# danpovey/quantization

Measured on AMD Instinct MI355X. Metric: vectors encoded/sec at dim=512, 8 codebooks; uint8 codes bit-exact vs ref, higher is better.
Workload: dtype f32 (products: exact 30-bit fixed point on the i8 MFMA); 1 GPU; Quantizer.encode, dim=512, bytes_per_frame=8, codebook_size=256, refine_indexes_iters=5, batch=65536 fp32 Gaussian vectors per GPU (BASELINE.json configs[1]), seeded synthetic codebooks; global_batch=65536, parallelism=batch-sharded x1, no collective

## Files before the change

include/mcq.h:

```cpp
#ifndef MCQ_H
#define MCQ_H

#include <stddef.h>
#include <stdint.h>

#ifdef __cplusplus
extern "C" {
#endif

#define MCQ_EINVAL (-1)
#define MCQ_EUNSUPPORTED (-2)
#define MCQ_EWORKSPACE (-3)

#define MCQ_ABI_VERSION 7
int mcq_abi_version(void);

int mcq_padded_dim(int D);

size_t mcq_prepared_bytes(int N, int K, int D);
size_t mcq_prepared_decode_bytes(int N, int K, int D);
size_t mcq_prepared_mean_offset(int N, int K, int D);
int mcq_prepare(const float *centers, float cscale_exp, const float *weight, const float *bias,
                int N, int K, int D, void *prepared, void *stream);

int mcq_prepare_dev(const float *centers, const float *scales_exp, const float *weight, const float *bias,
                    int N, int K, int D, void *prepared, void *stream);

int mcq_prepare_params(const float *centers, const float *centers_scale, const float *logits_scale, float speed,
                       const float *weight, const float *bias, int N, int K, int D, void *prepared,
                       float *scales_exp_out, void *stream);

size_t mcq_encode_workspace_bytes(long B, int N, int K, int D);
int mcq_encode(const float *x, long B, const void *prepared, float lscale_exp, int N, int K, int D,
               int refine_iters, uint8_t *out_u8, int64_t *out_i64, void *workspace,
               size_t workspace_bytes, void *stream);

#define MCQ_ENCODE_SKIP_FIXED_POINTS 1u
#define MCQ_ENCODE_ALL_PASSES 8u
#define MCQ_ENCODE_LSCALE_FROM_PREPARED 2u
#define MCQ_ENCODE_X_FP16 4u
int mcq_encode_ex(const float *x, long B, const void *prepared, float lscale_exp, int N, int K, int D,
                  int refine_iters, uint8_t *out_u8, int64_t *out_i64, void *workspace,
                  size_t workspace_bytes, void *stream, unsigned flags);

int mcq_refine_indexes(const float *x, long B, const void *prepared, int N, int K, int D, int refine_iters,
                       const int64_t *idx_in, int64_t *idx_out, void *workspace, size_t workspace_bytes,
                       void *stream);

int mcq_decode(const void *codes, int code_bytes, int codes_per_row, long B, const void *prepared,
               int N, int K, int D, float *out, void *stream);

int mcq_decode_backward(const float *grad_out, const int64_t *idx, long B, int N, int K, int D, float *gC,
                        void *stream);

int mcq_logits_argmax(const float *x, long B, const void *prepared, float lscale_exp, int N, int K, int D,
                      float *logits_out, int64_t *argmax_out, void *workspace, size_t workspace_bytes,
                      void *stream, unsigned flags);

int mcq_logits_refine(const float *x, long B, const void *prepared, float lscale_exp, int N, int K, int D,
                      int refine_iters, float *logits_out, int64_t *idx_out, void *workspace, size_t workspace_bytes,
                      void *stream, unsigned flags);
int mcq_logits_refine_codes(const float *x, long B, const void *prepared, float lscale_exp, int N, int K, int D,
                            int refine_iters, float *logits_out, int64_t *idx_out, uint8_t *codes_out, void *workspace,
// ... 81 lines not shown
```

quantization_amd/_lib.py:

```python
import ctypes
import os

_HERE = os.path.dirname(os.path.abspath(__file__))
_ALT = os.environ.get("MCQ_LIB_PATH") if os.environ.get("MCQ_ALLOW_LIB_PATH") == "1" else None
LIB_PATH = _ALT or os.path.join(_HERE, "lib", "libmcq_hip.so")

SYMBOLS = (
    "mcq_abi_version", "mcq_padded_dim", "mcq_prepared_bytes", "mcq_prepared_decode_bytes", "mcq_prepared_mean_offset", "mcq_prepare", "mcq_prepare_dev", "mcq_prepare_params", "mcq_encode_workspace_bytes",
    "mcq_encode", "mcq_encode_ex", "mcq_refine_indexes", "mcq_decode", "mcq_decode_backward", "mcq_logits", "mcq_logits_workspace_bytes", "mcq_last_encode_launches", "mcq_test_select", "mcq_profile_encode", "mcq_profile_category_name",
    "mcq_logits_argmax", "mcq_logits_refine", "mcq_logits_refine_codes", "mcq_loss_workspace_bytes", "mcq_loss_fwd", "mcq_loss_bwd", "mcq_recon_fwd", "mcq_loss_tail",
    "mcq_jcl_prefix_fwd", "mcq_jcl_prefix_bwd", "mcq_scatter_rows", "mcq_decode_backward_u8",
    "mcq_weight_grad", "mcq_weight_grad_workspace_bytes", "mcq_adam_step", "mcq_loss_head", "mcq_loss_head_tail", "mcq_scales_exp",
    "mcq_decode_backward_waves", "mcq_decode_backward_u8_ex", "mcq_loss_bwd_waves", "mcq_loss_bwd_ex", "mcq_grad_tail",
    "mcq_search_tables", "mcq_code_norms", "mcq_search_workspace_bytes", "mcq_search_scan",
    "mcq_search_scan_metric", "mcq_code_rnorms", "mcq_rnorms_from_norms",
)

MCQ_EINVAL, MCQ_EUNSUPPORTED, MCQ_EWORKSPACE = -1, -2, -3
MCQ_SEARCH_L2, MCQ_SEARCH_IP, MCQ_SEARCH_COS = 0, 1, 2
MCQ_ENCODE_ALL_PASSES = 8
_lib = None


class McqError(RuntimeError):
    pass


def lib():
    global _lib
    if _lib is not None:
        return _lib
    if not os.path.exists(LIB_PATH):
        raise McqError(f"{LIB_PATH} is missing: build it with `python -c 'import __graft_entry__ as g; g.build()'` "
                       "(hipcc --offload-arch=gfx950); quantization_amd has no CPU fallback")
    L = ctypes.CDLL(LIB_PATH)
    vp, f32, i32, i64, sz = ctypes.c_void_p, ctypes.c_float, ctypes.c_int, ctypes.c_long, ctypes.c_size_t
    L.mcq_abi_version.restype = i32
    L.mcq_padded_dim.restype = i32
    L.mcq_padded_dim.argtypes = [i32]
    L.mcq_prepared_bytes.restype = sz
    L.mcq_prepared_bytes.argtypes = [i32, i32, i32]
    L.mcq_prepared_decode_bytes.restype = sz
    L.mcq_prepared_decode_bytes.argtypes = [i32, i32, i32]
# ... 105 lines not shown
```

quantization_amd/csrc/mcq_api.hip:

```cpp
#include "../../include/mcq.h"
#include "mcq_kernels.h"
#include "mcq_fix_kernels.h"
#include "mcq_loss_kernels.h"
#include "mcq_tf_kernels.h"
#include "mcq_pass16_kernels.h"
#include "mcq_train_kernels.h"
#include "mcq_search_kernels.h"

#include <cstdlib>
#include <type_traits>
#include <utility>
#include <vector>

using namespace mcq;

namespace {

inline int round_up16(int d) { return (d + 15) & ~15; }
inline size_t align256(size_t v) { return (v + 255) & ~size_t(255); }
inline bool is_pow2(int v) { return v > 0 && (v & (v - 1)) == 0; }

int k_cutoff(int K, int L) {
    int kc = (K <= 16) ? 8 : 16;
    while (L >= 4) { L /= 4; kc *= 2; }
// ... 160 lines not shown
        (void)hipEventCreate(&e);
        (void)hipEventRecord(e, stream);
        ev.push_back(e);
        first.push_back(open);
        last.push_back((int)ev.size() - 1);
        cat.push_back(category);
        open = (int)ev.size() - 1;
    }
};

thread_local int g_last_launches = 0;

#define MCQ_LAUNCH_CHECK()                               \
    do {                                                 \
        hipError_t e_ = hipGetLastError();               \
        if (e_ != hipSuccess) return (int)e_;            \
        ++g_last_launches;                               \
    } while (0)

FixRowsArgs fix_rows_args(const float *src, int xh, long R, int D, long ld, int8_t *planes, int *exps, float *xx,
                          const float *bias_src = nullptr, float *bias_dst = nullptr, const float *sub = nullptr,
                          long sub_per = 0, long sub_ld = 0, const float *dot_vec = nullptr, float *dot_out = nullptr) {
    return FixRowsArgs{src, xh, R, fix_round_rows(R), D, ld, fix_round_cols(D), planes, exps, xx, bias_src, bias_dst,
                       sub, sub_per, sub_ld, dot_vec, dot_out};
}

int launch_fix_rows(const float *src, int xh, long R, int D, long ld, int8_t *planes, int *exps, float *xx, hipStream_t st,
                    const float *sub = nullptr) {
    const FixRowsArgs a = fix_rows_args(src, xh, R, D, ld, planes, exps, xx, nullptr, nullptr, sub, 0, 0);
    hipLaunchKernelGGL(k_fix_rows<4>, dim3((unsigned)(a.Rp / 4)), dim3(256), 0, st, a);
    MCQ_LAUNCH_CHECK();
    return 0;
}

int launch_fix_rows2(const FixRowsArgs &a, const FixRowsArgs &b, hipStream_t st) {
    const unsigned na = (unsigned)(a.Rp / 4), nb = (unsigned)(b.Rp / 4);
    hipLaunchKernelGGL(k_fix_rows2<4>, dim3(na + nb), dim3(256), 0, st, a, b, na);
    MCQ_LAUNCH_CHECK();
    return 0;
}

template <int MODE>
int launch_fgemm(FixGemm g, hipStream_t st) {
    static bool allowed[64] = {};
    int dev = 0;
    if (hipGetDevice(&dev) != hipSuccess || dev < 0 || dev >= 64) dev = 63;
    if (!allowed[dev] || dev == 63) {
        const hipError_t attr = hipFuncSetAttribute(reinterpret_cast<const void *>(&k_fgemm<MODE>),
                                                    hipFuncAttributeMaxDynamicSharedMemorySize, kFixLds);
        if (attr != hipSuccess) return (int)attr;
        allowed[dev] = true;
    }
    const long MT = g.RA / kFixTile, NT = g.RB / kFixTile;
    const int H = (MODE == FG_LOGITS && g.K > kFixTile) ? g.K / kFixTile : 1;
    const long big = g.walk_rows ? NT : MT, small_units = (g.walk_rows ? MT : NT) / H;
    long units = (big + 7) / 8 * small_units;
    if (units > 32) units = 32;
    hipLaunchKernelGGL((k_fgemm<MODE>), dim3((unsigned)(8 * units)), dim3(512), kFixLds, st, g);
    MCQ_LAUNCH_CHECK();
    return 0;
}

int launch_xc(const int8_t *xf, const int *xe, long B, const int8_t *Cf, const int *Ce, long nk, int D, float *out,
              hipStream_t st) {
    FixGemm g{};
    g.A = xf; g.ea = xe; g.RA = fix_round_rows(B); g.M = B;
    g.B = Cf; g.eb = Ce; g.RB = fix_round_rows(nk); g.N = nk;
    g.Dq = fix_round_cols(D);
    g.walk_rows = 0;
    g.out = out; g.ldo = nk;
    return launch_fgemm<FG_STORE>(g, st);
}

int launch_logits(const int8_t *xf, const int *xe, long B, const Prepared &P, int N, int K, int D, float lscale,
                  const float *lscale_ptr, float *logits, void *idx, hipStream_t st) {
    const long nk = (long)N * K;
    FixGemm g{};
    g.A = P.Wf; g.ea = P.We; g.RA = fix_round_rows(nk); g.M = nk;
    g.B = xf; g.eb = xe; g.RB = fix_round_rows(B); g.N = B;
    g.Dq = fix_round_cols(D);
    g.walk_rows = 1;
    g.bias = P.bias; g.wmu = P.wmu; g.lscale = lscale; g.lscale_ptr = lscale_ptr;
    g.logits = logits; g.ldo = nk; g.idx = idx; g.idx_wide = K > 256 ? 1 : 0; g.K = K; g.ncb = N;
    return launch_fgemm<FG_LOGITS>(g, st);
}

constexpr unsigned kCapStage0 = 32768, kCapWave = 65536;
inline unsigned pass_grid(unsigned full, bool capped, unsigned cap) { return (capped && full > cap) ? cap : full; }

template <int K>
int launch_tf_stage0_k(int N, const float *G, const float *XC, const tf_code_of<K> *idx, const float *R, const float *Q, long B,
                       int keep, tf_code_of<K> *ent, float *S, tf_code_of<K> *fin, const int *nact, const int *map, hipStream_t st,
                       bool capped) {
    const unsigned vgrid = (unsigned)(((B + 3) / 4) * N);
    const dim3 grid(pass_grid(vgrid, capped, kCapStage0)), block(256);
#define MCQ_S0_CASE(NN)                                                                                                            \
    case NN:                                                                                                                       \
        if (capped) hipLaunchKernelGGL((k_tf_stage0<K, NN, true>), grid, block, 0, st, G, XC, idx, R, Q, B, keep, ent, S, fin, nact, map, vgrid); \
        else hipLaunchKernelGGL((k_tf_stage0<K, NN, false>), grid, block, 0, st, G, XC, idx, R, Q, B, keep, ent, S, fin, nact, map, vgrid);      \
        break;
    switch (N) {
        MCQ_S0_CASE(1) MCQ_S0_CASE(2) MCQ_S0_CASE(4) MCQ_S0_CASE(8) MCQ_S0_CASE(16) MCQ_S0_CASE(32) MCQ_S0_CASE(64)
        default: return MCQ_EUNSUPPORTED;
    }
#undef MCQ_S0_CASE
    MCQ_LAUNCH_CHECK();
    return 0;
// ... 221 lines not shown
                 uint8_t *codes_also ) {
    g_last_launches = 0;
    if (!domain_ok(N, K, D)) return domain_err(N, K, D);
    if (B < 0 || iters < 0 || iters > 60 || (out_u8 == nullptr) == (out_i64 == nullptr)) return MCQ_EINVAL;
    if (sizeof(CT) > 1 && (out_u8 != nullptr || codes_also != nullptr)) return MCQ_EINVAL;
    if (B == 0) return 0;
    if (!x || !prepared || !workspace) return MCQ_EINVAL;
    const size_t per = workspace_per_vector(N, K, D), slack = workspace_slack(D);
    if (workspace_bytes < slack + per) return MCQ_EWORKSPACE;
    long chunk = (long)((workspace_bytes - slack) / per);
    if (chunk > B) chunk = B;
    if (chunk < B && chunk < 128) return MCQ_EWORKSPACE;
    if (chunk < B) chunk &= ~127L;
    const Prepared P = prepared_view(prepared, N, K, D);
    const int pack = (out_u8 != nullptr && K == 16 && N >= 2) ? 2 : 1;
    const bool want_skip = (flags & MCQ_ENCODE_ALL_PASSES) == 0 && iters >= 3;

    for (long lo = 0; lo < B; lo += chunk) {
        const long Bc = (B - lo < chunk) ? (B - lo) : chunk;
        const WorkspaceT<CT> w = carve<CT>(workspace, Bc, N, K, D);
        const int xh = (flags & MCQ_ENCODE_X_FP16) ? 1 : 0;
        const float *xc = xh ? reinterpret_cast<const float *>(reinterpret_cast<const uint16_t *>(x) + lo * D) : x + lo * D;
        int rc;
        if (init_idx == nullptr || iters > 0) {
            if (prof) prof->begin(CAT_XX);
            rc = launch_fix_rows(xc, xh, Bc, D, D, w.xf, w.xe, w.xx, st, P.mean);
            if (rc) return rc;
            if (prof) prof->end(CAT_XX);
        }
        if (init_idx != nullptr) {
            hipLaunchKernelGGL(k_import_indexes<CT>, dim3((unsigned)((Bc * N + 255) / 256)), dim3(256), 0, st,
                               init_idx + lo * N, Bc * N, K, w.idx);
            MCQ_LAUNCH_CHECK();
            if (prof) prof->untimed();
        } else {
            if (prof) prof->begin(CAT_LOGITS);
            rc = launch_logits(w.xf, w.xe, Bc, P, N, K, D, lscale,
                               (flags & MCQ_ENCODE_LSCALE_FROM_PREPARED) ? P.scales + 1 : nullptr,
                               logits_out ? logits_out + lo * N * K : nullptr, w.idx, st);
            if (rc) return rc;
            if (prof) prof->end(CAT_LOGITS);
        }
        if (iters > 0) {
            if (prof) prof->begin(CAT_XC);
            rc = launch_xc(w.xf, w.xe, Bc, P.Cf, P.Ce, (long)N * K, D, w.XC, st);
            if (rc) return rc;
            if (prof) prof->end(CAT_XC);
        }
        const bool use_p16 = sizeof(CT) == 1 && K == 16 && (N == 16 || N == 8) && iters > 0 && prof == nullptr && pass16_enabled();
        const bool skip = want_skip && !use_p16 && Bc >= skip_min_batch();
        int iters_left = iters;
        CT *idx_cur = w.idx, *idx_new = skip ? w.idxB : w.idx, *idx_pk = w.idxC;
        const int *map_cur = nullptr, *nact = nullptr;
        int *map_nxt = w.map[0], *map_spare = w.map[1];
        float *E_cur = w.E, *R_cur = w.R, *E_alt = w.gterms, *R_alt = w.gterms + ((Bc + 3) & ~3L);
        if (skip) {
            hipLaunchKernelGGL(k_zero_counts, dim3(1), dim3(64), 0, st, w.cnt, 64);
            MCQ_LAUNCH_CHECK();
            if (prof) prof->untimed();
        }
        bool wrote_direct = false;
        if constexpr (sizeof(CT) == 1) {
// ... 971 lines not shown
```

quantization_amd/csrc/mcq_fix_kernels.h:

```cpp
#pragma once
#include "mcq_kernels.h"

namespace mcq {

typedef int i32x4 __attribute__((ext_vector_type(4)));
typedef int i32x16 __attribute__((ext_vector_type(16)));

constexpr int kFixTile = 128;
constexpr int kFixColPad = 128;
constexpr int kFixRing = 4;
constexpr int kFixSlot = 32768;
constexpr int kFixOperand = 16384;
constexpr int kFixInfo = kFixRing * kFixSlot;
constexpr int kFixLds = kFixInfo + 4096;

__host__ __device__ inline long fix_round_rows(long r) { return (r + kFixTile - 1) / kFixTile * kFixTile; }
__host__ __device__ inline int fix_round_cols(int d) { return (d + kFixColPad - 1) / kFixColPad * kFixColPad; }
__host__ __device__ inline size_t fix_plane_bytes(long R, int D) { return (size_t)fix_round_rows(R) * fix_round_cols(D) * 4; }

__device__ __forceinline__ int fix_q(float v, int e) {
    float s = ldexpf(v, 30 - e);
    s = fminf(fmaxf(s, -1073741824.0f), 1073741824.0f);
    return (int)rintf(s);
}

struct FixRowsArgs {
    const float *src;
    int xh;
    long R, Rp;
    int D;
    long ld;
    int Dq;
    int8_t *planes;
    int *exps;
    float *xx;
    const float *bias_src;
    float *bias_dst;
    const float *sub;
    long sub_per, sub_ld;
    const float *dot_vec;
    float *dot_out;
};

template <int RW, bool DOT>
__device__ __forceinline__ void fix_rows_body(const FixRowsArgs &a, unsigned bid) {
    const float *__restrict__ src = a.src;
    const int xh = a.xh, D = a.D, Dq = a.Dq;
    const long R = a.R, Rp = a.Rp, ld = a.ld;
    float *__restrict__ xx = a.xx;
    const float *__restrict__ bias_src = a.bias_src;
    float *__restrict__ bias_dst = a.bias_dst;
    const float *__restrict__ sub = a.sub;
    int8_t *__restrict__ planes = a.planes;
    constexpr int RPW = RW / 4;
    __shared__ __attribute__((aligned(16))) unsigned tile[128 * RW * 4];
    __shared__ int es[RW];
    const int tid = threadIdx.x, lane = tid & 63, wave = tid >> 6;
    const long row0 = (long)bid * RW;
    if (bias_src && tid < RW && row0 + tid < R) bias_dst[row0 + tid] = bias_src[row0 + tid];
    const _Float16 *srch = reinterpret_cast<const _Float16 *>(src);
    const bool vec_ok = ((ld & 3) == 0) && ((D & 3) == 0) && ((reinterpret_cast<uintptr_t>(src) & (xh ? 7 : 15)) == 0);
    auto load4 = [&](long row, int q) -> f32x4 {
        f32x4 v = {0.f, 0.f, 0.f, 0.f};
        if (row >= R || 4 * q >= D) return v;
        if (vec_ok) return xh ? load_h4(srch + row * ld + 4 * q) : *reinterpret_cast<const f32x4 *>(src + row * ld + 4 * q);
#pragma unroll
        for (int c = 0; c < 4; ++c)
            if (4 * q + c < D) v[c] = xh ? (float)srch[row * ld + 4 * q + c] : src[row * ld + 4 * q + c];
        return v;
    };
    auto vec4 = [&](const float *p, int q) -> f32x4 {
        f32x4 v = {0.f, 0.f, 0.f, 0.f};
        if (4 * q >= D) return v;
        if (((D & 3) == 0) && ((reinterpret_cast<uintptr_t>(p) & 15) == 0)) return *reinterpret_cast<const f32x4 *>(p + 4 * q);
#pragma unroll
        for (int c = 0; c < 4; ++c)
            if (4 * q + c < D) v[c] = p[4 * q + c];
        return v;
    };
    auto sub4 = [&](long row, int q) -> f32x4 {
        if (!sub || row >= R) return f32x4{0.f, 0.f, 0.f, 0.f};
        return vec4(sub + (a.sub_per ? (row / a.sub_per) * a.sub_ld : 0), q);
// ... 123 lines not shown
                t4[i] = t;
            }
            const long row = row0 + RPW * wave + rr;
            if (lane == 0 && row < R) {
                float tt = (float)t4[3];
                tt = __builtin_fmaf((float)t4[2], 256.0f, tt);
                tt = __builtin_fmaf((float)t4[1], 65536.0f, tt);
                tt = __builtin_fmaf((float)t4[0], 16777216.0f, tt);
                a.dot_out[row] = ldexpf(tt, es[RPW * wave + rr] + ev - 36);
            }
        }
    }
}

template <int RW>
__global__ void __launch_bounds__(256) k_fix_rows(const FixRowsArgs a) { fix_rows_body<RW, false>(a, blockIdx.x); }

template <int RW>
__global__ void __launch_bounds__(256) k_fix_rows2(const FixRowsArgs a, const FixRowsArgs b, unsigned blocks_a) {
    if (blockIdx.x < blocks_a) fix_rows_body<RW, false>(a, blockIdx.x);
    else fix_rows_body<RW, true>(b, blockIdx.x - blocks_a);
}

enum { FG_STORE = 0, FG_LOGITS = 1 };

struct FixGemm {
    const int8_t *A, *B;
    const int *ea, *eb;
    long RA, RB;
    long M, N;
    int Dq;
    int walk_rows;
    float *out;
    long ldo;
    const float *bias;
    const float *wmu;
    const float *lscale_ptr;
    float lscale;
    float *logits;
    void *idx;
    int idx_wide;
    int K, ncb;
};

__device__ __forceinline__ void fg_store_idx(const FixGemm &g, long pos, long entry) {
    if (g.idx_wide) static_cast<uint16_t *>(g.idx)[pos] = (uint16_t)entry;
    else static_cast<uint8_t *>(g.idx)[pos] = (uint8_t)entry;
}

template <int MODE>
__global__ void __launch_bounds__(512)
k_fgemm(const FixGemm g) {
    extern __shared__ __attribute__((aligned(16))) char smem[];
    const int tid = threadIdx.x, lane = tid & 63, wave = tid >> 6;
    const int wm = wave & 1, wn = wave >> 1;
    const int r32 = lane & 31, kh = lane >> 5;
    const long MT = g.RA / kFixTile, NT = g.RB / kFixTile;
    const int H = (MODE == FG_LOGITS && g.K > kFixTile) ? g.K / kFixTile : 1;
    const long big = g.walk_rows ? NT : MT, small_units = (g.walk_rows ? MT : NT) / H;
    const int xcd = blockIdx.x & 7, slot = blockIdx.x >> 3, per_xcd = gridDim.x >> 3;
    auto tile_of = [&](long t, long &m0, long &n0) -> bool {
        const long unit = t / H, half = t % H;
        const long idx = slot + unit * per_xcd;
        const long bt = (idx / small_units) * 8 + xcd, st = (idx % small_units) * H + half;
        m0 = (g.walk_rows ? st : bt) * kFixTile;
        n0 = (g.walk_rows ? bt : st) * kFixTile;
        return bt < big;
    };
    i32x16 acc[2][4];
    const int nst = g.Dq / 32;
    const int wu = __builtin_amdgcn_readfirstlane(wave);
    const int op = wu >> 2, chunk = (wu >> 1) & 1, half = wu & 1;
    const long R = op ? g.RB : g.RA;
    const long pl = R * 16, sstride = 8 * R * 16;
    const unsigned dbase = (unsigned)(size_t)smem + op * kFixOperand + (4 * chunk) * 2048 + half * 1024;
    const unsigned voff = lane * 16, voff4 = lane * 4;
    auto base_of = [&](long m0, long n0) { return (op ? g.B + n0 * 16 : g.A + m0 * 16) + (long)(4 * chunk) * R * 16 + half * 1024; };
    auto issue1 = [&](const int8_t *p, int st, int g4) {
        const int8_t *pg = p + g4 * pl;
        const unsigned d = dbase + (st % kFixRing) * kFixSlot + g4 * 2048;
        asm volatile(
            "s_mov_b32 m0, %[d]\n\ts_nop 0\n\t"
            "global_load_lds_dwordx4 %[vo], %[p]\n\t"
            :
            : [vo] "v"(voff), [p] "s"(pg), [d] "s"(d)
            : "memory");
    };
    auto issue_info = [&](long m0, long n0) {
        if (wu < (MODE == FG_LOGITS ? 8 : 4)) {
            const void *src = wu < 2 ? static_cast<const void *>(g.ea + m0 + 64 * wu)
                                     : (wu < 4 ? static_cast<const void *>(g.eb + n0 + 64 * (wu - 2))
                                               : (wu < 6 ? static_cast<const void *>(g.bias + m0 + 64 * (wu - 4))
                                                         : static_cast<const void *>(g.wmu + m0 + 64 * (wu - 6))));
            const unsigned d = (unsigned)(size_t)smem + kFixInfo + 256 * (wu < 6 ? wu : wu + 4);
            asm volatile(
                "s_mov_b32 m0, %[d]\n\ts_nop 0\n\t"
                "global_load_lds_dword %[vo], %[p]\n\t"
                :
                : [vo] "v"(voff4), [p] "s"(src), [d] "s"(d)
                : "memory");
        }
    };
    long m0, n0, m0n = 0, n0n = 0;
    if (!tile_of(0, m0, n0)) return;
    const int8_t *pcur = base_of(m0, n0), *pnext = pcur;
    auto step = [&](int st, const i32x4 (&a)[2][4], const i32x4 (&b)[4], i32x4 (&an)[2][4], i32x4 (&bn)[4]) {
        const char *base = smem + ((st + 1) % kFixRing) * kFixSlot;
        const int8_t *p = (st + 4 < nst) ? pcur + (st + 4) * sstride : pnext + (st + 4 - nst) * sstride;
        constexpr int PI[10] = {0, 0, 1, 0, 1, 2, 0, 1, 2, 3};
        constexpr int PJ[10] = {0, 1, 0, 2, 1, 0, 3, 2, 1, 0};
        constexpr int LO[5] = {0, 3, 6, 8, 10};
#pragma unroll
        for (int g4 = 0; g4 < 4; ++g4) {
            issue1(p, st, g4);
#pragma unroll
            for (int t = 0; t < 2; ++t)
                an[t][g4] = *reinterpret_cast<const i32x4 *>(base + (kh * 4 + g4) * 2048 + (64 * wm + 32 * t + r32) * 16);
            bn[g4] = *reinterpret_cast<const i32x4 *>(base + kFixOperand + (kh * 4 + g4) * 2048 + (32 * wn + r32) * 16);
#pragma unroll
            for (int q = LO[g4]; q < LO[g4 + 1]; ++q)
#pragma unroll
                for (int ta = 0; ta < 2; ++ta)
                    acc[ta][PI[q] + PJ[q]] =
                        __builtin_amdgcn_mfma_i32_32x32x32_i8(a[ta][PI[q]], b[PJ[q]], acc[ta][PI[q] + PJ[q]], 0, 0, 0);
            __builtin_amdgcn_sched_barrier(0);
        }
    };
    i32x4 a0[2][4], b0[4], a1[2][4], b1[4];
    issue_info(m0, n0);
#pragma unroll
    for (int q = 0; q < 4; ++q)
#pragma unroll
        for (int g4 = 0; g4 < 4; ++g4) issue1(pcur + q * sstride, q, g4);
    asm volatile("s_waitcnt vmcnt(12)" ::: "memory");
    __builtin_amdgcn_s_barrier();
#pragma unroll
    for (int l = 0; l < 4; ++l) {
#pragma unroll
        for (int t = 0; t < 2; ++t)
            a0[t][l] = *reinterpret_cast<const i32x4 *>(smem + (kh * 4 + l) * 2048 + (64 * wm + 32 * t + r32) * 16);
        b0[l] = *reinterpret_cast<const i32x4 *>(smem + kFixOperand + (kh * 4 + l) * 2048 + (32 * wn + r32) * 16);
    }
    int *info = reinterpret_cast<int *>(smem + kFixInfo);
    float *infof = reinterpret_cast<float *>(smem + kFixInfo);
    float runv = 0.f;
    int runk = 0;
    for (long t = 0;; ++t) {
        const bool has_next = tile_of(t + 1, m0n, n0n);
        pnext = has_next ? base_of(m0n, n0n) : pcur;
#pragma unroll
        for (int a = 0; a < 2; ++a)
#pragma unroll
            for (int s = 0; s < 4; ++s)
#pragma unroll
                for (int v = 0; v < 16; ++v) acc[a][s][v] = 0;
        for (int st = 0; st < nst; st += 2) {
            asm volatile("s_waitcnt vmcnt(8)\n\ts_waitcnt lgkmcnt(0)" ::: "memory");
            __builtin_amdgcn_s_barrier();
            step(st, a0, b0, a1, b1);
            asm volatile("s_waitcnt vmcnt(8)\n\ts_waitcnt lgkmcnt(0)" ::: "memory");
            __builtin_amdgcn_s_barrier();
            step(st + 1, a1, b1, a0, b0);
        }
        auto value = [&](int ta, int v, int e) -> float {
            float tt = (float)acc[ta][3][v];
            tt = __builtin_fmaf((float)acc[ta][2][v], 256.0f, tt);
            tt = __builtin_fmaf((float)acc[ta][1][v], 65536.0f, tt);
            tt = __builtin_fmaf((float)acc[ta][0][v], 16777216.0f, tt);
            return ldexpf(tt, e);
        };
        int rbase = 64 * wm + 4 * kh, cbase = 32 * wn + r32;
        asm volatile("" : "+v"(rbase), "+v"(cbase));
        i32x4 er[2][4];
#pragma unroll
        for (int ta = 0; ta < 2; ++ta)
#pragma unroll
            for (int q = 0; q < 4; ++q) er[ta][q] = *reinterpret_cast<const i32x4 *>(&info[rbase + 32 * ta + 8 * q]);
        const bool full = (m0 + kFixTile <= g.M) && (n0 + kFixTile <= g.N);
        const int ecol = info[128 + cbase] - 36;
        const int rows_left = (int)((g.M - m0 - rbase) > 128 ? 128 : (g.M - m0 - rbase));
        if (MODE == FG_STORE) {
            const bool col_ok = n0 + cbase < g.N;
            float *orow = g.out + (m0 + rbase) * g.ldo + n0 + cbase;
            if (full) {
#pragma unroll
                for (int ta = 0; ta < 2; ++ta)
#pragma unroll
                    for (int v = 0; v < 16; ++v) {
                        const int ro = 32 * ta + 8 * (v >> 2) + (v & 3);
                        orow[(long)ro * g.ldo] = value(ta, v, er[ta][v >> 2][v & 3] + ecol);
                    }
            } else {
#pragma unroll
                for (int ta = 0; ta < 2; ++ta)
#pragma unroll
                    for (int v = 0; v < 16; ++v) {
                        const int ro = 32 * ta + 8 * (v >> 2) + (v & 3);
                        const float val = value(ta, v, er[ta][v >> 2][v & 3] + ecol);
                        if (col_ok && ro < rows_left) orow[(long)ro * g.ldo] = val;
                    }
            }
        } else {
            const float ls = g.lscale_ptr ? *g.lscale_ptr : g.lscale;
            float bv[4];
            int bk[4];
            const long col = n0 + cbase;
            float *lrow = g.logits ? g.logits + col * g.ldo + m0 + rbase : nullptr;
#pragma unroll
            for (int ta = 0; ta < 2; ++ta) {
#pragma unroll
                for (int v4 = 0; v4 < 4; ++v4) {
                    const f32x4 br4 = *reinterpret_cast<const f32x4 *>(&infof[256 + rbase + 32 * ta + 8 * v4]);
                    const f32x4 wm4 = *reinterpret_cast<const f32x4 *>(&infof[640 + rbase + 32 * ta + 8 * v4]);
                    f32x4 q4;
#pragma unroll
                    for (int c = 0; c < 4; ++c) {
                        const int v = 4 * v4 + c;
                        const int rl = rbase + 32 * ta + 8 * v4 + c;
                        const float val = __fadd_rn(__fmul_rn(__fadd_rn(value(ta, v, er[ta][v4][c] + ecol), wm4[c]), ls), br4[c]);
                        q4[c] = val;
                        const int gi = 2 * ta + (v4 >> 1);
                        if ((v4 & 1) == 0 && c == 0) { bv[gi] = val; bk[gi] = rl; }
                        else if (val > bv[gi]) { bv[gi] = val; bk[gi] = rl; }
// ... 35 lines not shown
                        const int hf = (int)(t % H);
                        float v = bv[0];
                        long k = m0 + bk[0];
                        if (better(exv[cbase], exk[cbase], bv[0], bk[0])) { v = exv[cbase]; k = m0 + exk[cbase]; }
                        if (hf > 0 && !(v > runv)) { v = runv; k = runk; }
                        runv = v;
                        runk = (int)k;
                        if (hf == H - 1 && col < g.N && k < g.M) fg_store_idx(g, col * g.ncb + k / K, k % K);
                    }
                }
            }
        }
        if (!has_next) break;
        asm volatile("s_waitcnt lgkmcnt(0)" ::: "memory");
        __builtin_amdgcn_s_barrier();
        m0 = m0n;
        n0 = n0n;
        pcur = pnext;
        issue_info(m0, n0);
    }
    asm volatile("s_waitcnt vmcnt(0)" ::: "memory");
}

}
```

quantization_amd/quantizer.py:

```python
import binascii
import ctypes
import math
import os
import weakref

import torch
from torch import Tensor, nn

from . import _lib


_param_epoch = [0]
_quantizer_params = {}
_optimizer_hits = weakref.WeakKeyDictionary()


def _note_optimizer_step(optimizer, *_args, **_kwargs):
    try:
        nparams = sum(len(g["params"]) for g in optimizer.param_groups)
        known = _optimizer_hits.get(optimizer)
        if known is None or known[0] != nparams or known[2] != len(_quantizer_params):
            hit = False
            for g in optimizer.param_groups:
                for q in g["params"]:
# ... 32 lines not shown
def _scale_exp(scale: Tensor, speed: float) -> float:
    return float((scale.detach().to("cpu", torch.float32) * speed).exp())


class Quantizer(nn.Module):

    def __init__(self, dim: int, codebook_size: int, num_codebooks: int):
        super().__init__()
        assert _is_pow2(codebook_size)
        assert _is_pow2(num_codebooks)
        self.dim = dim
        self.codebook_size = codebook_size
        self.num_codebooks = num_codebooks
        self.to_logits = nn.Linear(dim, codebook_size * num_codebooks)
        self.centers = nn.Parameter(
            self.to_logits.weight.detach().clone().reshape(num_codebooks, codebook_size, dim))
        self.logits_scale = nn.Parameter(torch.zeros(()))
        self.centers_scale = nn.Parameter(torch.zeros(()))
        self.scale_speed = 10.0
        id_bytes = binascii.b2a_hex(os.urandom(4))
        self.id_str = id_bytes.decode("utf-8")
        self.register_buffer("id_buf", torch.tensor(list(id_bytes), dtype=torch.uint8))
        self.skip_fixed_points = True
        self._pinned_scales = None
        self._prep = None
        self._ws = None

    def __getstate__(self):
        st = super().__getstate__() if hasattr(super(), "__getstate__") else self.__dict__.copy()
        st = dict(st)
        st["_prep"] = None
        st["_ws"] = None
        st.pop("_host_stage", None)
        return st

    def _current_prep(self):
        if self._prep is None:
            raise RuntimeError("no derived state: call Quantizer._prepared() before reading its scale factors")
        return self._prep

    @property
    def _scale_flags(self) -> int:
        return self._current_prep().scale_flags

    @property
    def _lscale_exp(self) -> float:
# ... 135 lines not shown
                                "(no CPU fallback)")
        L = _lib.lib()
        N, K, D = self.num_codebooks, self.codebook_size, self.dim
        x_fp16 = x2d.dtype == torch.float16
        x2d = x2d.detach().contiguous() if x_fp16 else x2d.detach().to(torch.float32).contiguous()
        B = x2d.shape[0]
        dev = x2d.device
        with torch.no_grad():
            blob = self._prepared()
        pack = 2 if (as_bytes and K == 16 and N >= 2) else 1
        if as_bytes:
            out = torch.empty((B, N // pack), dtype=torch.uint8, device=dev)
        else:
            out = torch.empty((B, N), dtype=torch.int64, device=dev)
        if B == 0:
            return out
        ws = self._workspace(B, dev)
        with torch.cuda.device(dev):
            st = torch.cuda.current_stream(dev).cuda_stream
            rc = L.mcq_encode_ex(x2d.data_ptr(), B, blob.data_ptr(), self._lscale_exp, N, K, D, int(iters),
                                 out.data_ptr() if as_bytes else None, None if as_bytes else out.data_ptr(),
                                 ws.data_ptr(), ws.numel(), st,
                                 (0 if getattr(self, "skip_fixed_points", True) else _lib.MCQ_ENCODE_ALL_PASSES) | self._scale_flags |
                                 (4 if x_fp16 else 0))
        _lib.check(rc, "mcq_encode")
        return out

    def encode(self, x: Tensor, refine_indexes_iters: int = 5, as_bytes: bool = True) -> Tensor:
        x2d = x.reshape(-1, self.dim)
        if as_bytes:
            assert self.codebook_size <= 256
        codes = self._search(x2d, refine_indexes_iters, as_bytes)
        return codes.reshape(*x.shape[:-1], codes.shape[-1])

    def encode_from_host(self, x: Tensor, refine_indexes_iters: int = 5, as_bytes: bool = True,
                         chunk: int = 32768) -> Tensor:
        dev = self.centers.device
        if dev.type != "cuda":
            raise _lib.McqError("quantization_amd.Quantizer runs on a HIP device only")
        x2d = x.reshape(-1, self.dim)
        if x2d.dtype != torch.float16:
            x2d = x2d.to(torch.float32)
        if not x2d.is_pinned():
            x2d = x2d.contiguous().pin_memory()
        B = x2d.shape[0]
        pack = 2 if (as_bytes and self.codebook_size == 16 and self.num_codebooks >= 2) else 1
        width = self.num_codebooks // pack
# ... 489 lines not shown
```

Before: 14.16 million vectors/s.

## Screen logits argmax with truncated limb product and exact recheck of close calls

After: 14.38 million vectors/s (median of 6 runs). 1.02x the previous value.

```diff
diff --git a/include/mcq.h b/include/mcq.h
--- a/include/mcq.h
+++ b/include/mcq.h
@@ -39,6 +39,7 @@
 #define MCQ_ENCODE_ALL_PASSES 8u
 #define MCQ_ENCODE_LSCALE_FROM_PREPARED 2u
 #define MCQ_ENCODE_X_FP16 4u
+#define MCQ_ENCODE_EXACT_LOGITS 16u
 int mcq_encode_ex(const float *x, long B, const void *prepared, float lscale_exp, int N, int K, int D,
                   int refine_iters, uint8_t *out_u8, int64_t *out_i64, void *workspace,
                   size_t workspace_bytes, void *stream, unsigned flags);
diff --git a/quantization_amd/_lib.py b/quantization_amd/_lib.py
--- a/quantization_amd/_lib.py
+++ b/quantization_amd/_lib.py
@@ -19,6 +19,7 @@
 MCQ_EINVAL, MCQ_EUNSUPPORTED, MCQ_EWORKSPACE = -1, -2, -3
 MCQ_SEARCH_L2, MCQ_SEARCH_IP, MCQ_SEARCH_COS = 0, 1, 2
 MCQ_ENCODE_ALL_PASSES = 8
+MCQ_ENCODE_EXACT_LOGITS = 16
 _lib = None
 
 
diff --git a/quantization_amd/csrc/mcq_api.hip b/quantization_amd/csrc/mcq_api.hip
--- a/quantization_amd/csrc/mcq_api.hip
+++ b/quantization_amd/csrc/mcq_api.hip
@@ -206,12 +206,13 @@
                           const float *bias_src = nullptr, float *bias_dst = nullptr, const float *sub = nullptr,
                           long sub_per = 0, long sub_ld = 0, const float *dot_vec = nullptr, float *dot_out = nullptr) {
     return FixRowsArgs{src, xh, R, fix_round_rows(R), D, ld, fix_round_cols(D), planes, exps, xx, bias_src, bias_dst,
-                       sub, sub_per, sub_ld, dot_vec, dot_out};
+                       sub, sub_per, sub_ld, dot_vec, dot_out, nullptr};
 }
 
 int launch_fix_rows(const float *src, int xh, long R, int D, long ld, int8_t *planes, int *exps, float *xx, hipStream_t st,
-                    const float *sub = nullptr) {
-    const FixRowsArgs a = fix_rows_args(src, xh, R, D, ld, planes, exps, xx, nullptr, nullptr, sub, 0, 0);
+                    const float *sub = nullptr, unsigned *clear = nullptr) {
+    FixRowsArgs a = fix_rows_args(src, xh, R, D, ld, planes, exps, xx, nullptr, nullptr, sub, 0, 0);
+    a.clear = clear;
     hipLaunchKernelGGL(k_fix_rows<4>, dim3((unsigned)(a.Rp / 4)), dim3(256), 0, st, a);
     MCQ_LAUNCH_CHECK();
     return 0;
@@ -227,20 +228,21 @@
 template <int MODE>
 int launch_fgemm(FixGemm g, hipStream_t st) {
     static bool allowed[64] = {};
+    constexpr int lds = MODE == FG_SCREEN ? kFixLdsScreen : kFixLds;
     int dev = 0;
     if (hipGetDevice(&dev) != hipSuccess || dev < 0 || dev >= 64) dev = 63;
     if (!allowed[dev] || dev == 63) {
         const hipError_t attr = hipFuncSetAttribute(reinterpret_cast<const void *>(&k_fgemm<MODE>),
-                                                    hipFuncAttributeMaxDynamicSharedMemorySize, kFixLds);
+                                                    hipFuncAttributeMaxDynamicSharedMemorySize, lds);
         if (attr != hipSuccess) return (int)attr;
         allowed[dev] = true;
     }
     const long MT = g.RA / kFixTile, NT = g.RB / kFixTile;
-    const int H = (MODE == FG_LOGITS && g.K > kFixTile) ? g.K / kFixTile : 1;
+    const int H = (MODE != FG_STORE && g.K > kFixTile) ? g.K / kFixTile : 1;
     const long big = g.walk_rows ? NT : MT, small_units = (g.walk_rows ? MT : NT) / H;
     long units = (big + 7) / 8 * small_units;
     if (units > 32) units = 32;
-    hipLaunchKernelGGL((k_fgemm<MODE>), dim3((unsigned)(8 * units)), dim3(512), kFixLds, st, g);
+    hipLaunchKernelGGL((k_fgemm<MODE>), dim3((unsigned)(8 * units)), dim3(512), lds, st, g);
     MCQ_LAUNCH_CHECK();
     return 0;
 }
@@ -256,8 +258,14 @@
     return launch_fgemm<FG_STORE>(g, st);
 }
 
+inline bool exact_logits_forced() {
+    static const bool on = getenv("MCQ_EXACT_LOGITS") && atoi(getenv("MCQ_EXACT_LOGITS")) != 0;
+    return on;
+}
+
 int launch_logits(const int8_t *xf, const int *xe, long B, const Prepared &P, int N, int K, int D, float lscale,
-                  const float *lscale_ptr, float *logits, void *idx, hipStream_t st) {
+                  const float *lscale_ptr, float *logits, void *idx, hipStream_t st, unsigned *und_cnt = nullptr,
+                  unsigned *und_list = nullptr) {
     const long nk = (long)N * K;
     FixGemm g{};
     g.A = P.Wf; g.ea = P.We; g.RA = fix_round_rows(nk); g.M = nk;
@@ -266,7 +274,19 @@
     g.walk_rows = 1;
     g.bias = P.bias; g.wmu = P.wmu; g.lscale = lscale; g.lscale_ptr = lscale_ptr;
     g.logits = logits; g.ldo = nk; g.idx = idx; g.idx_wide = K > 256 ? 1 : 0; g.K = K; g.ncb = N;
-    return launch_fgemm<FG_LOGITS>(g, st);
+    if (und_cnt == nullptr) return launch_fgemm<FG_LOGITS>(g, st);
+    if (logits != nullptr) return MCQ_EINVAL;
+    g.und_cnt = und_cnt; g.und_list = und_list; g.und_cap = (unsigned)(B * N);
+    const int rc = launch_fgemm<FG_SCREEN>(g, st);
+    if (rc) return rc;
+    FixRecheck r{};
+    r.W = P.Wf; r.X = xf; r.ew = P.We; r.ex = xe; r.RW = g.RA; r.RX = g.RB; r.Dq = g.Dq;
+    r.bias = P.bias; r.wmu = P.wmu; r.lscale_ptr = lscale_ptr; r.lscale = lscale;
+    r.idx = idx; r.idx_wide = g.idx_wide; r.K = K; r.ncb = N; r.cnt = und_cnt; r.list = und_list; r.cap = g.und_cap;
+    const long waves = B * N;
+    hipLaunchKernelGGL(k_fscreen_recheck, dim3((unsigned)(waves < 4096 ? (waves + 3) / 4 : 1024)), dim3(256), 0, st, r);
+    MCQ_LAUNCH_CHECK();
+    return 0;
 }
 
 constexpr unsigned kCapStage0 = 32768, kCapWave = 65536;
@@ -534,9 +554,12 @@
         const int xh = (flags & MCQ_ENCODE_X_FP16) ? 1 : 0;
         const float *xc = xh ? reinterpret_cast<const float *>(reinterpret_cast<const uint16_t *>(x) + lo * D) : x + lo * D;
         int rc;
+        const bool screen = init_idx == nullptr && logits_out == nullptr && (flags & MCQ_ENCODE_EXACT_LOGITS) == 0 &&
+                            !exact_logits_forced() && (size_t)Bc * N < ((size_t)1 << 31);
+        unsigned *const und_cnt = reinterpret_cast<unsigned *>(w.cnt + 63), *const und_list = reinterpret_cast<unsigned *>(w.XC);
         if (init_idx == nullptr || iters > 0) {
             if (prof) prof->begin(CAT_XX);
-            rc = launch_fix_rows(xc, xh, Bc, D, D, w.xf, w.xe, w.xx, st, P.mean);
+            rc = launch_fix_rows(xc, xh, Bc, D, D, w.xf, w.xe, w.xx, st, P.mean, screen ? und_cnt : nullptr);
             if (rc) return rc;
             if (prof) prof->end(CAT_XX);
         }
@@ -549,7 +572,7 @@
             if (prof) prof->begin(CAT_LOGITS);
             rc = launch_logits(w.xf, w.xe, Bc, P, N, K, D, lscale,
                                (flags & MCQ_ENCODE_LSCALE_FROM_PREPARED) ? P.scales + 1 : nullptr,
-                               logits_out ? logits_out + lo * N * K : nullptr, w.idx, st);
+                               logits_out ? logits_out + lo * N * K : nullptr, w.idx, st, screen ? und_cnt : nullptr, und_list);
             if (rc) return rc;
             if (prof) prof->end(CAT_LOGITS);
         }
diff --git a/quantization_amd/csrc/mcq_fix_kernels.h b/quantization_amd/csrc/mcq_fix_kernels.h
--- a/quantization_amd/csrc/mcq_fix_kernels.h
+++ b/quantization_amd/csrc/mcq_fix_kernels.h
@@ -13,6 +13,7 @@
 constexpr int kFixOperand = 16384;
 constexpr int kFixInfo = kFixRing * kFixSlot;
 constexpr int kFixLds = kFixInfo + 4096;
+constexpr int kFixLdsScreen = kFixLds + 1024;
 
 __host__ __device__ inline long fix_round_rows(long r) { return (r + kFixTile - 1) / kFixTile * kFixTile; }
 __host__ __device__ inline int fix_round_cols(int d) { return (d + kFixColPad - 1) / kFixColPad * kFixColPad; }
@@ -40,6 +41,7 @@
     long sub_per, sub_ld;
     const float *dot_vec;
     float *dot_out;
+    unsigned *clear;
 };
 
 template <int RW, bool DOT>
@@ -58,6 +60,7 @@
     const int tid = threadIdx.x, lane = tid & 63, wave = tid >> 6;
     const long row0 = (long)bid * RW;
     if (bias_src && tid < RW && row0 + tid < R) bias_dst[row0 + tid] = bias_src[row0 + tid];
+    if (a.clear && bid == 0 && tid == 0) *a.clear = 0u;
     const _Float16 *srch = reinterpret_cast<const _Float16 *>(src);
     const bool vec_ok = ((ld & 3) == 0) && ((D & 3) == 0) && ((reinterpret_cast<uintptr_t>(src) & (xh ? 7 : 15)) == 0);
     auto load4 = [&](long row, int q) -> f32x4 {
@@ -227,7 +230,7 @@
     else fix_rows_body<RW, true>(b, blockIdx.x - blocks_a);
 }
 
-enum { FG_STORE = 0, FG_LOGITS = 1 };
+enum { FG_STORE = 0, FG_LOGITS = 1, FG_SCREEN = 2 };
 
 struct FixGemm {
     const int8_t *A, *B;
@@ -246,6 +249,8 @@
     void *idx;
     int idx_wide;
     int K, ncb;
+    unsigned *und_cnt, *und_list;
+    unsigned und_cap;
 };
 
 __device__ __forceinline__ void fg_store_idx(const FixGemm &g, long pos, long entry) {
@@ -257,11 +262,13 @@
 __global__ void __launch_bounds__(512)
 k_fgemm(const FixGemm g) {
     extern __shared__ __attribute__((aligned(16))) char smem[];
+    constexpr bool SCREEN = MODE == FG_SCREEN, LOGITS = MODE != FG_STORE;
+    constexpr int NL = SCREEN ? 3 : 4;
     const int tid = threadIdx.x, lane = tid & 63, wave = tid >> 6;
     const int wm = wave & 1, wn = wave >> 1;
     const int r32 = lane & 31, kh = lane >> 5;
     const long MT = g.RA / kFixTile, NT = g.RB / kFixTile;
-    const int H = (MODE == FG_LOGITS && g.K > kFixTile) ? g.K / kFixTile : 1;
+    const int H = (LOGITS && g.K > kFixTile) ? g.K / kFixTile : 1;
     const long big = g.walk_rows ? NT : MT, small_units = (g.walk_rows ? MT : NT) / H;
     const int xcd = blockIdx.x & 7, slot = blockIdx.x >> 3, per_xcd = gridDim.x >> 3;
     auto tile_of = [&](long t, long &m0, long &n0) -> bool {
@@ -272,7 +279,7 @@
         n0 = (g.walk_rows ? bt : st) * kFixTile;
         return bt < big;
     };
-    i32x16 acc[2][4];
+    i32x16 acc[2][NL];
     const int nst = g.Dq / 32;
     const int wu = __builtin_amdgcn_readfirstlane(wave);
     const int op = wu >> 2, chunk = (wu >> 1) & 1, half = wu & 1;
@@ -292,7 +299,7 @@
             : "memory");
     };
     auto issue_info = [&](long m0, long n0) {
-        if (wu < (MODE == FG_LOGITS ? 8 : 4)) {
+        if (wu < (LOGITS ? 8 : 4)) {
             const void *src = wu < 2 ? static_cast<const void *>(g.ea + m0 + 64 * wu)
                                      : (wu < 4 ? static_cast<const void *>(g.eb + n0 + 64 * (wu - 2))
                                                : (wu < 6 ? static_cast<const void *>(g.bias + m0 + 64 * (wu - 4))
@@ -309,14 +316,14 @@
     long m0, n0, m0n = 0, n0n = 0;
     if (!tile_of(0, m0, n0)) return;
     const int8_t *pcur = base_of(m0, n0), *pnext = pcur;
-    auto step = [&](int st, const i32x4 (&a)[2][4], const i32x4 (&b)[4], i32x4 (&an)[2][4], i32x4 (&bn)[4]) {
+    auto step = [&](int st, const i32x4 (&a)[2][NL], const i32x4 (&b)[NL], i32x4 (&an)[2][NL], i32x4 (&bn)[NL]) {
         const char *base = smem + ((st + 1) % kFixRing) * kFixSlot;
         const int8_t *p = (st + 4 < nst) ? pcur + (st + 4) * sstride : pnext + (st + 4 - nst) * sstride;
         constexpr int PI[10] = {0, 0, 1, 0, 1, 2, 0, 1, 2, 3};
         constexpr int PJ[10] = {0, 1, 0, 2, 1, 0, 3, 2, 1, 0};
-        constexpr int LO[5] = {0, 3, 6, 8, 10};
-#pragma unroll
-        for (int g4 = 0; g4 < 4; ++g4) {
+        constexpr int LO[5] = {0, SCREEN ? 2 : 3, SCREEN ? 4 : 6, SCREEN ? 6 : 8, 10};
+#pragma unroll
+        for (int g4 = 0; g4 < NL; ++g4) {
             issue1(p, st, g4);
 #pragma unroll
             for (int t = 0; t < 2; ++t)
@@ -331,16 +338,17 @@
             __builtin_amdgcn_sched_barrier(0);
         }
     };
-    i32x4 a0[2][4], b0[4], a1[2][4], b1[4];
+    i32x4 a0[2][NL], b0[NL], a1[2][NL], b1[NL];
     issue_info(m0, n0);
 #pragma unroll
     for (int q = 0; q < 4; ++q)
 #pragma unroll
-        for (int g4 = 0; g4 < 4; ++g4) issue1(pcur + q * sstride, q, g4);
-    asm volatile("s_waitcnt vmcnt(12)" ::: "memory");
+        for (int g4 = 0; g4 < NL; ++g4) issue1(pcur + q * sstride, q, g4);
+    if constexpr (SCREEN) asm volatile("s_waitcnt vmcnt(9)" ::: "memory");
+    else asm volatile("s_waitcnt vmcnt(12)" ::: "memory");
     __builtin_amdgcn_s_barrier();
 #pragma unroll
-    for (int l = 0; l < 4; ++l) {
+    for (int l = 0; l < NL; ++l) {
 #pragma unroll
         for (int t = 0; t < 2; ++t)
             a0[t][l] = *reinterpret_cast<const i32x4 *>(smem + (kh * 4 + l) * 2048 + (64 * wm + 32 * t + r32) * 16);
@@ -350,26 +358,31 @@
     float *infof = reinterpret_cast<float *>(smem + kFixInfo);
     float runv = 0.f;
     int runk = 0;
+    float runs = 0.f, runt = 0.f, runq = 0.f;
+    int runj = 0, rune = 0;
     for (long t = 0;; ++t) {
         const bool has_next = tile_of(t + 1, m0n, n0n);
         pnext = has_next ? base_of(m0n, n0n) : pcur;
 #pragma unroll
         for (int a = 0; a < 2; ++a)
 #pragma unroll
-            for (int s = 0; s < 4; ++s)
+            for (int s = 0; s < NL; ++s)
 #pragma unroll
                 for (int v = 0; v < 16; ++v) acc[a][s][v] = 0;
         for (int st = 0; st < nst; st += 2) {
-            asm volatile("s_waitcnt vmcnt(8)\n\ts_waitcnt lgkmcnt(0)" ::: "memory");
+            if constexpr (SCREEN) asm volatile("s_waitcnt vmcnt(6)\n\ts_waitcnt lgkmcnt(0)" ::: "memory");
+            else asm volatile("s_waitcnt vmcnt(8)\n\ts_waitcnt lgkmcnt(0)" ::: "memory");
             __builtin_amdgcn_s_barrier();
             step(st, a0, b0, a1, b1);
-            asm volatile("s_waitcnt vmcnt(8)\n\ts_waitcnt lgkmcnt(0)" ::: "memory");
+            if constexpr (SCREEN) asm volatile("s_waitcnt vmcnt(6)\n\ts_waitcnt lgkmcnt(0)" ::: "memory");
+            else asm volatile("s_waitcnt vmcnt(8)\n\ts_waitcnt lgkmcnt(0)" ::: "memory");
             __builtin_amdgcn_s_barrier();
             step(st + 1, a1, b1, a0, b0);
         }
         auto value = [&](int ta, int v, int e) -> float {
-            float tt = (float)acc[ta][3][v];
-            tt = __builtin_fmaf((float)acc[ta][2][v], 256.0f, tt);
+            float tt;
+            if constexpr (SCREEN) tt = __fmul_rn((float)acc[ta][2][v], 256.0f);
+            else tt = __builtin_fmaf((float)acc[ta][2][v], 256.0f, (float)acc[ta][NL - 1][v]);
             tt = __builtin_fmaf((float)acc[ta][1][v], 65536.0f, tt);
             tt = __builtin_fmaf((float)acc[ta][0][v], 16777216.0f, tt);
             return ldexpf(tt, e);
@@ -404,6 +417,117 @@
                         const float val = value(ta, v, er[ta][v >> 2][v & 3] + ecol);
                         if (col_ok && ro < rows_left) orow[(long)ro * g.ldo] = val;
                     }
+            }
+        } else if constexpr (SCREEN) {
+            const float ls = g.lscale_ptr ? *g.lscale_ptr : g.lscale;
+            float bv[4], sv[4], tv[4], qm = 0.f;
+            int bk[4], sk[4];
+            const long col = n0 + cbase;
+#pragma unroll
+            for (int ta = 0; ta < 2; ++ta) {
+#pragma unroll
+                for (int v4 = 0; v4 < 4; ++v4) {
+                    const f32x4 br4 = *reinterpret_cast<const f32x4 *>(&infof[256 + rbase + 32 * ta + 8 * v4]);
+                    const f32x4 wm4 = *reinterpret_cast<const f32x4 *>(&infof[640 + rbase + 32 * ta + 8 * v4]);
+#pragma unroll
+                    for (int c = 0; c < 4; ++c) {
+                        const int v = 4 * v4 + c;
+                        const int rl = rbase + 32 * ta + 8 * v4 + c;
+                        const float s2 = __fmul_rn(__fadd_rn(value(ta, v, er[ta][v4][c] + ecol), wm4[c]), ls);
+                        const float val = __fadd_rn(s2, br4[c]);
+                        qm = fmaxf(qm, fmaxf(fabsf(s2), fabsf(val)));
+                        const int gi = 2 * ta + (v4 >> 1);
+                        if ((v4 & 1) == 0 && c == 0) { bv[gi] = val; bk[gi] = sk[gi] = rl; sv[gi] = tv[gi] = -INFINITY; }
+                        else {
+                            const bool c1 = val > bv[gi], c2 = val > sv[gi];
+                            tv[gi] = __builtin_amdgcn_fmed3f(tv[gi], sv[gi], val);
+                            sv[gi] = __builtin_amdgcn_fmed3f(sv[gi], bv[gi], val);
+                            sk[gi] = c1 ? bk[gi] : (c2 ? rl : sk[gi]);
+                            bk[gi] = c1 ? rl : bk[gi];
+                            bv[gi] = fmaxf(bv[gi], val);
+                        }
+                    }
+                }
+            }
+            int em = info[lane] > info[lane + 64] ? info[lane] : info[lane + 64];
+            for (int s = 32; s >= 1; s >>= 1) { const int o = __shfl_xor(em, s, 64); em = o > em ? o : em; }
+            auto merge = [](float &b1, int &k1, float &s1, int &j1, float &t1, float b2, int k2, float s2, int j2, float t2) {
+                if (b2 > b1) {
+                    float f = b1; b1 = b2; b2 = f;
+                    f = s1; s1 = s2; s2 = f;
+                    t1 = t2;
+                    int i = k1; k1 = k2; k2 = i;
+                    j1 = j2;
+                }
+                if (b2 > s1) { t1 = fmaxf(s1, s2); s1 = b2; j1 = k2; }
+                else t1 = fmaxf(t1, b2);
+            };
+            const float cA = 16.5f * 16384.0f * (float)g.Dq;
+            auto undecided = [&](float v, float s, float q, int e) {
+                const float margin = __fadd_rn(__fadd_rn(__fmul_rn(ldexpf(cA, e + ecol), ls), __fmul_rn(q, 1.9073486328125e-6f)), 7.5231638452626401e-37f);
+                return !(__fsub_rn(v, s) > margin);
+            };
+            auto append = [&](long pos, unsigned second_entry, bool many) {
+                const unsigned at = atomicAdd(g.und_cnt, 1u);
+                if (at < g.und_cap) {
+                    g.und_list[2 * (size_t)at] = (unsigned)pos;
+                    g.und_list[2 * (size_t)at + 1] = second_entry | (many ? 0x80000000u : 0u);
+                }
+            };
+            const int K = g.K;
+#pragma unroll
+            for (int gi = 0; gi < 4; ++gi)
+                merge(bv[gi], bk[gi], sv[gi], sk[gi], tv[gi], __shfl_xor(bv[gi], 32, 64), __shfl_xor(bk[gi], 32, 64),
+                      __shfl_xor(sv[gi], 32, 64), __shfl_xor(sk[gi], 32, 64), __shfl_xor(tv[gi], 32, 64));
+            qm = fmaxf(qm, __shfl_xor(qm, 32, 64));
+            if (K >= 32) {
+                merge(bv[0], bk[0], sv[0], sk[0], tv[0], bv[1], bk[1], sv[1], sk[1], tv[1]);
+                merge(bv[2], bk[2], sv[2], sk[2], tv[2], bv[3], bk[3], sv[3], sk[3], tv[3]);
+            }
+            if (K >= 64) merge(bv[0], bk[0], sv[0], sk[0], tv[0], bv[2], bk[2], sv[2], sk[2], tv[2]);
+            if (K <= 64) {
+                if (kh == 0) {
+                    const int span = K / 16;
+#pragma unroll
+                    for (int gi = 0; gi < 4; ++gi) {
+                        const long row = m0 + bk[gi];
+                        if ((gi % span) == 0 && col < g.N && row < g.M) {
+                            fg_store_idx(g, col * g.ncb + row / K, row % K);
+                            if (undecided(bv[gi], sv[gi], qm, em))
+                                append(col * g.ncb + row / K, (unsigned)((m0 + sk[gi]) % K), undecided(bv[gi], tv[gi], qm, em));
+                        }
+                    }
+                }
+            } else {
+                float *exv = infof + 384, *exs = infof + 768, *exq = infof + 896;
+                int *exk = info + 384 + 128;
+                float *ext = reinterpret_cast<float *>(smem + kFixInfo + 4096);
+                int *exj = reinterpret_cast<int *>(smem + kFixInfo + 4096 + 512);
+                if (wm == 1 && kh == 0) {
+                    exv[cbase] = bv[0]; exk[cbase] = bk[0]; exs[cbase] = sv[0]; exq[cbase] = qm;
+                    ext[cbase] = tv[0]; exj[cbase] = sk[0];
+                }
+                asm volatile("s_waitcnt lgkmcnt(0)" ::: "memory");
+                __builtin_amdgcn_s_barrier();
+                if (wm == 0 && kh == 0) {
+                    const int hf = (int)(t % H);
+                    float v = bv[0], s = sv[0], t3 = tv[0], q = fmaxf(qm, exq[cbase]);
+                    int kk = bk[0], jj = sk[0];
+                    merge(v, kk, s, jj, t3, exv[cbase], exk[cbase], exs[cbase], exj[cbase], ext[cbase]);
+                    kk += (int)m0;
+                    jj += (int)m0;
+                    if (hf > 0) {
+                        merge(v, kk, s, jj, t3, runv, runk, runs, runj, runt);
+                        q = fmaxf(q, runq);
+                        em = em > rune ? em : rune;
+                    }
+                    runv = v; runk = kk; runs = s; runj = jj; runt = t3; runq = q; rune = em;
+                    const long k = kk;
+                    if (hf == H - 1 && col < g.N && k < g.M) {
+                        fg_store_idx(g, col * g.ncb + k / K, k % K);
+                        if (undecided(v, s, q, em)) append(col * g.ncb + k / K, (unsigned)(jj % K), undecided(v, t3, q, em));
+                    }
+                }
             }
         } else {
             const float ls = g.lscale_ptr ? *g.lscale_ptr : g.lscale;
@@ -485,4 +609,86 @@
     asm volatile("s_waitcnt vmcnt(0)" ::: "memory");
 }
 
+struct FixRecheck {
+    const int8_t *W, *X;
+    const int *ew, *ex;
+    long RW, RX;
+    int Dq;
+    const float *bias, *wmu, *lscale_ptr;
+    float lscale;
+    void *idx;
+    int idx_wide;
+    int K, ncb;
+    const unsigned *cnt, *list;
+    unsigned cap;
+};
+
+__global__ void __launch_bounds__(256) k_fscreen_recheck(const FixRecheck a) {
+    const int lane = threadIdx.x & 63;
+    const unsigned wv = __builtin_amdgcn_readfirstlane(blockIdx.x * 4 + (threadIdx.x >> 6)), nwv = gridDim.x * 4;
+    unsigned n = *a.cnt;
+    n = n < a.cap ? n : a.cap;
+    const float ls = a.lscale_ptr ? *a.lscale_ptr : a.lscale;
+    const int K = a.K, nch = a.Dq / 16;
+    for (unsigned i = wv; i < n; i += nwv) {
+        const unsigned pos = a.list[2 * (size_t)i], snd = a.list[2 * (size_t)i + 1];
+        const long col = pos / (unsigned)a.ncb;
+        const int cb = (int)(pos % (unsigned)a.ncb);
+        const int ecol = a.ex[col] - 36;
+        auto chunk = [&](int (&T)[4], int c, long row) {
+            i32x4 xl[4], wl[4];
+#pragma unroll
+            for (int l = 0; l < 4; ++l) {
+                xl[l] = *reinterpret_cast<const i32x4 *>(a.X + (((long)c * 4 + l) * a.RX + col) * 16);
+                wl[l] = *reinterpret_cast<const i32x4 *>(a.W + (((long)c * 4 + l) * a.RW + row) * 16);
+            }
+#pragma unroll
+            for (int p = 0; p < 4; ++p)
+#pragma unroll
+                for (int q = 0; p + q < 4; ++q)
+#pragma unroll
+                    for (int d = 0; d < 4; ++d) T[p + q] = __builtin_amdgcn_sdot4(wl[p][d], xl[q][d], T[p + q], false);
+        };
+        auto logit = [&](const int (&T)[4], long row) -> float {
+            float tt = (float)T[3];
+            tt = __builtin_fmaf((float)T[2], 256.0f, tt);
+            tt = __builtin_fmaf((float)T[1], 65536.0f, tt);
+            tt = __builtin_fmaf((float)T[0], 16777216.0f, tt);
+            return __fadd_rn(__fmul_rn(__fadd_rn(ldexpf(tt, a.ew[row] + ecol), a.wmu[row]), ls), a.bias[row]);
+        };
+        float bv = -INFINITY;
+        int bk = 0x7fffffff;
+        if ((snd & 0x80000000u) == 0) {
+            const int first = a.idx_wide ? (int)static_cast<const uint16_t *>(a.idx)[pos] : (int)static_cast<const uint8_t *>(a.idx)[pos];
+            const int j = (lane < 32) ? first : (int)snd;
+            const long row = (long)cb * K + j;
+            int T[4] = {0, 0, 0, 0};
+            for (int c = lane & 31; c < nch; c += 32) chunk(T, c, row);
+#pragma unroll
+            for (int p = 0; p < 4; ++p)
+                for (int sft = 16; sft >= 1; sft >>= 1) T[p] += __shfl_xor(T[p], sft, 64);
+            bv = logit(T, row);
+            bk = j;
+        } else {
+            for (int j = lane; j < K; j += 64) {
+                const long row = (long)cb * K + j;
+                int T[4] = {0, 0, 0, 0};
+#pragma unroll 4
+                for (int c = 0; c < nch; ++c) chunk(T, c, row);
+                const float val = logit(T, row);
+                if (j == lane || val > bv) { bv = val; bk = j; }
+            }
+        }
+        for (int s = 32; s >= 1; s >>= 1) {
+            const float ov = __shfl_xor(bv, s, 64);
+            const int ok = __shfl_xor(bk, s, 64);
+            if ((ov > bv) | ((ov == bv) & (ok < bk))) { bv = ov; bk = ok; }
+        }
+        if (lane == 0) {
+            if (a.idx_wide) static_cast<uint16_t *>(a.idx)[pos] = (uint16_t)bk;
+            else static_cast<uint8_t *>(a.idx)[pos] = (uint8_t)bk;
+        }
+    }
 }
+
+}
diff --git a/quantization_amd/quantizer.py b/quantization_amd/quantizer.py
--- a/quantization_amd/quantizer.py
+++ b/quantization_amd/quantizer.py
@@ -78,6 +78,7 @@
         self.id_str = id_bytes.decode("utf-8")
         self.register_buffer("id_buf", torch.tensor(list(id_bytes), dtype=torch.uint8))
         self.skip_fixed_points = True
+        self.exact_logits = False
         self._pinned_scales = None
         self._prep = None
         self._ws = None
@@ -259,7 +260,7 @@
                                  out.data_ptr() if as_bytes else None, None if as_bytes else out.data_ptr(),
                                  ws.data_ptr(), ws.numel(), st,
                                  (0 if getattr(self, "skip_fixed_points", True) else _lib.MCQ_ENCODE_ALL_PASSES) | self._scale_flags |
-                                 (4 if x_fp16 else 0))
+                                 (4 if x_fp16 else 0) | (_lib.MCQ_ENCODE_EXACT_LOGITS if getattr(self, "exact_logits", False) else 0))
         _lib.check(rc, "mcq_encode")
         return out
 
```
